# adrelino/mv-lm-icp

Hardware: NVIDIA H100
Metric: ICP iterations/sec (corr+LM) (higher is better)
Workload: dtype f64

## Files before the change

mv_lm_icp_b200/csrc/lm_step.cuh:

```cuda
#pragma once
#include <cuda_runtime.h>
#include "../../include/mvicp.h"
#include "se3_math.cuh"
#include "types.cuh"

namespace mv {

constexpr int STEP_THREADS = 512;
constexpr int EOUT = 160;

struct LmState {
  mvicp_lm_options opt;
  int32_t param, cost_kind, robust, M, E, F, n, G;
  int32_t phase, done, termination, iteration, n_success, n_invalid, n_evals, n_solves, reuse_diagonal, nonrigid;
  double radius, decrease_factor, x_cost, cand_cost, x_norm, initial_cost, model_cost_change, step_norm, gmax;
};

struct NormalLayout {
  const int32_t* col;
  const int32_t* hb_ptr; const int32_t* hb_row; const int32_t* hb_col; const int32_t* hc_edge; const int32_t* hc_sub; int32_t n_hblocks;
  const int32_t* gb_ptr; const int32_t* gc_edge; const int32_t* gc_side;
  const int32_t* rlast; const int32_t* rfirst;
  const int32_t* rowbase;
  double *Lg, *rhs;
  int32_t l_in_smem;
};

struct LmWork {
  LmState* S;
  const EdgeDev* edges;
  const double* eout;
  volatile int* peer_flags;
  int32_t world, xseq;
  double* x;
  double* cand;
  Rt* Rt_eval;
  double* K_eval;
  FrameGen* G_eval;
  double* poses16;
  volatile int32_t* host_flag;
  int32_t seq;
  long long* prof;
};

struct LmProblem {
  LmState* S;
  const int32_t* frame;
  const int32_t* edge;
  NormalLayout lay;
  double *H, *g, *Hc, *gc, *scale, *diag, *step;
};

__device__ __forceinline__ double block_sum(double v, double* red) {
  __syncthreads();
  const int lane = threadIdx.x & 31, wid = threadIdx.x >> 5;
#pragma unroll
  for (int o = 16; o > 0; o >>= 1) v += __shfl_down_sync(0xffffffffu, v, o);
  if (lane == 0) red[wid] = v;
  __syncthreads();
  if (threadIdx.x == 0) { double s = 0; for (int w = 0; w < STEP_THREADS / 32; ++w) s += red[w]; red[32] = s; }
  __syncthreads();
  return red[32];
}
__device__ __forceinline__ double block_max(double v, double* red) {
  __syncthreads();
  const int lane = threadIdx.x & 31, wid = threadIdx.x >> 5;
#pragma unroll
  for (int o = 16; o > 0; o >>= 1) v = fmax(v, __shfl_down_sync(0xffffffffu, v, o));
  if (lane == 0) red[wid] = v;
  __syncthreads();
  if (threadIdx.x == 0) { double s = 0; for (int w = 0; w < STEP_THREADS / 32; ++w) s = fmax(s, red[w]); red[32] = s; }
  __syncthreads();
  return red[32];
}

__device__ __forceinline__ void gather_blocks(const NormalLayout& l, const double* eout, int n, double* H) {
  for (int idx = threadIdx.x; idx < l.n_hblocks * 36; idx += blockDim.x) {
    const int b = idx / 36, r = idx - 36 * b, i = r / 6, j = r - 6 * i;
    double s = 0;
    for (int c = l.hb_ptr[b]; c < l.hb_ptr[b + 1]; ++c) {
      const int e = l.hc_edge[c], sub = l.hc_sub[c];
      s += eout[(size_t)EOUT * e + (6 * (sub >> 1) + i) * 12 + 6 * (sub & 1) + j];
    }
    H[(size_t)(l.hb_row[b] + i) * n + l.hb_col[b] + j] = s;
  }
}
__device__ __forceinline__ void gather_gradient(const NormalLayout& l, const double* eout, int M, double* g) {
  for (int idx = threadIdx.x; idx < M * 6; idx += blockDim.x) {
    const int f = idx / 6, i = idx - 6 * f;
    if (l.col[f] < 0) continue;
    double s = 0;
    for (int c = l.gb_ptr[f]; c < l.gb_ptr[f + 1]; ++c) s += eout[(size_t)EOUT * l.gc_edge[c] + 144 + 6 * l.gc_side[c] + i];
    g[l.col[f] + i] = s;
  }
}
__device__ __forceinline__ double edge_cost_sum(const double* eout, int E, double* red, const int32_t* edge = nullptr) {
  double s = 0.0;
  for (int e = threadIdx.x; e < E; e += blockDim.x) s += eout[(size_t)EOUT * (edge ? edge[e] : e) + 156];
  return block_sum(s, red);
}
template <typename State> __device__ __forceinline__ void copy_state(State* dst, const State* src) {
  for (int i = threadIdx.x; i < (int)(sizeof(State) / sizeof(int32_t)); i += blockDim.x)
    reinterpret_cast<int32_t*>(dst)[i] = reinterpret_cast<const int32_t*>(src)[i];
  __syncthreads();
}
__device__ __forceinline__ void publish_step(volatile int32_t* host_flag, int32_t seq, bool done) {
  __threadfence();
  host_flag[seq & 7] = (seq << 1) | (done ? 1 : 0);
  __threadfence_system();
}

__global__ void lm_init_kernel(LmWork w) {
  LmState* S = w.S;
  const int f = blockIdx.x * blockDim.x + threadIdx.x;
  if (f >= S->M) return;
  double x[7] = {0, 0, 0, 0, 0, 0, 0};
  param_of_pose(S->param, w.poses16 + 16 * f, x);
  if (S->param != PARAM_AA) {
    const double n2 = x[0] * x[0] + x[1] * x[1] + x[2] * x[2] + x[3] * x[3];
    if (!(fabs(n2 - 1.0) <= 1e-9)) atomicExch(&S->nonrigid, 1);
  }
  Rt a; Rt_of_param(S->param, x, &a);
  double K[36]; tangent_map(S->param, x, &a, K);
  for (int i = 0; i < 7; ++i) { w.x[7 * f + i] = x[i]; w.cand[7 * f + i] = x[i]; }
  w.Rt_eval[f] = a;
  for (int i = 0; i < 36; ++i) w.K_eval[36 * f + i] = K[i];
  if (w.G_eval && S->param != PARAM_AA) frame_general(S->param, x, &w.G_eval[f]);
}

__device__ __forceinline__ void chol_factor_diag(double* L, const int32_t* rb, int j0, double* dinv, volatile int* s_ok, int lane) {
  double D[6][6], inv[6];
#pragma unroll
  for (int i = 0; i < 6; ++i)
#pragma unroll
    for (int k = 0; k <= i; ++k) D[i][k] = L[rb[j0 + i] + j0 + k];
  bool okb = true;
#pragma unroll
  for (int k = 0; k < 6; ++k) {
    double d = D[k][k];
#pragma unroll
    for (int m = 0; m < k; ++m) d -= D[k][m] * D[k][m];
    if (!(d > 0.0) || !isfinite(d)) okb = false;
    inv[k] = rsqrt(d); D[k][k] = d * inv[k];
#pragma unroll
    for (int i = k + 1; i < 6; ++i) {
      double v = D[i][k];
#pragma unroll
      for (int m = 0; m < k; ++m) v -= D[i][m] * D[k][m];
      D[i][k] = v * inv[k];
    }
  }
  __syncwarp();
  if (lane == 0) {
    if (!okb) *s_ok = 0;
#pragma unroll
    for (int i = 0; i < 6; ++i) {
#pragma unroll
      for (int k = 0; k <= i; ++k) L[rb[j0 + i] + j0 + k] = D[i][k];
      dinv[j0 + i] = inv[i];
    }
  }
}

__device__ bool chol_solve(double* L, const int32_t* __restrict__ rowbase, int n, double* scratch, double* dinv, double* y,
                           const int32_t* __restrict__ rlast, const int32_t* __restrict__ rfirst, long long* prof = nullptr) {
  const int T = blockDim.x, tid = threadIdx.x, lane = tid & 31, wid = tid >> 5, nw = T >> 5;
  int32_t* s_rfirst = reinterpret_cast<int32_t*>(scratch);
  int32_t* s_rlast = s_rfirst + n;
  int32_t* rb = s_rlast + n;
  volatile int* s_ok = reinterpret_cast<volatile int*>(rb + n + 1);
  for (int i = tid; i < n; i += T) { s_rfirst[i] = rfirst[i]; s_rlast[i] = rlast[i]; }
  for (int i = tid; i <= n; i += T) rb[i] = rowbase[i];
  if (tid == 0) *s_ok = 1;
  __syncthreads();
  const int NB = n / 6;
  if (wid == 0) chol_factor_diag(L, rb, 0, dinv, s_ok, lane);
  __syncthreads();
  long long t_panel = 0, t_ahead = 0, t_bar = 0;
  for (int J = 0; J < NB; ++J) {
    if (!*s_ok) return false;
    const long long c0 = prof ? clock64() : 0;
    const int j0 = 6 * J;
    const int rl = s_rlast[j0 + 5];
    const int nrows = rl - (j0 + 5) + 1;
    for (int q = tid; q < nrows; q += T) {
      const int r = (q == nrows - 1) ? n : j0 + 6 + q;
      if (r < n && s_rfirst[r] > j0 + 5) continue;
      double* row = L + rb[r] + j0;
      double v[6];
#pragma unroll
      for (int k = 0; k < 6; ++k) {
        double a = row[k];
#pragma unroll
        for (int m = 0; m < k; ++m) a -= v[m] * L[rb[j0 + k] + j0 + m];
        v[k] = a * dinv[j0 + k];
      }
#pragma unroll
      for (int k = 0; k < 6; ++k) row[k] = v[k];
    }
    const long long c1 = prof ? clock64() : 0;
    __syncthreads();
    const long long c2 = prof ? clock64() : 0;
    const bool next = J + 1 < NB;
    if (wid == 0 && next) {
      const int b0 = j0 + 6;
      if (lane < 21 && s_rfirst[b0] <= j0 + 5) {
        int i = 0, rem = lane; while (rem > i) { rem -= i + 1; ++i; }
        const int k = rem;
        double* row = L + rb[b0 + i]; const double* lc = L + rb[b0 + k] + j0;
        double a = row[b0 + k];
#pragma unroll
        for (int m = 0; m < 6; ++m) a -= row[j0 + m] * lc[m];
        row[b0 + k] = a;
      }
      __syncwarp();
      chol_factor_diag(L, rb, b0, dinv, s_ok, lane);
    } else {
      const int w0 = next ? 1 : 0, wn = next ? nw - 1 : nw;
      const int qfirst = next ? 6 : 0;
      for (int q = qfirst + (wid - w0); q < nrows; q += wn) {
        const int r = (q == nrows - 1) ? n : j0 + 6 + q;
        if (r < n && s_rfirst[r] > j0 + 5) continue;
        double* row = L + rb[r];
        double lr[6];
#pragma unroll
        for (int k = 0; k < 6; ++k) lr[k] = row[j0 + k];
        const int cend = min(r, rl);
        for (int c = j0 + 6 + lane; c <= cend; c += 32) {
          if (s_rfirst[c] > j0 + 5) continue;
          const double* lc = L + rb[c] + j0;
          double a = row[c];
#pragma unroll
          for (int k = 0; k < 6; ++k) a -= lr[k] * lc[k];
          row[c] = a;
        }
      }
    }
    const long long c3 = prof ? clock64() : 0;
    __syncthreads();
    if (prof) { const long long c4 = clock64(); t_panel += c1 - c0; t_ahead += c3 - c2; t_bar += (c2 - c1) + (c4 - c3); }
  }
  if (prof && tid == 0) { prof[8] = t_panel; prof[9] = t_ahead; prof[10] = t_bar; }
  if (!*s_ok) return false;
  for (int i = tid; i < n; i += T) y[i] = L[rb[n] + i];
  __syncthreads();
  if (wid == 0) {
    for (int J = NB - 1; J >= 0; --J) {
      const int j0 = 6 * J;
      double x[6];
#pragma unroll
      for (int k = 5; k >= 0; --k) {
        double a = y[j0 + k];
#pragma unroll
        for (int m = k + 1; m < 6; ++m) a -= L[rb[j0 + m] + j0 + k] * x[m];
        x[k] = a * dinv[j0 + k];
      }
      __syncwarp();
#pragma unroll
      for (int k = 0; k < 6; ++k) if (lane == k) y[j0 + k] = x[k];
      for (int i = s_rfirst[j0] + lane; i < j0; i += 32) {
        double a = y[i];
#pragma unroll
        for (int k = 0; k < 6; ++k) a -= L[rb[j0 + k] + i] * x[k];
        y[i] = a;
      }
      __syncwarp();
    }
  }
  __syncthreads();
  return true;
}

__device__ __forceinline__ void lm_step_body(const LmWork& w, const LmProblem& p) {
  extern __shared__ double smem[];
  __shared__ double red[40];
  __shared__ int s_flag;
  if (p.S->done) return;
  const int tid = threadIdx.x, T = blockDim.x;
  __shared__ LmState s_state;
  copy_state(&s_state, p.S);
  LmState* S = &s_state;
  const int n = S->n, M = S->M, E = S->E, param = S->param;
  const NormalLayout& lay = p.lay;
  long long* prof = w.prof ? w.prof + 16 * (w.seq & 3) : nullptr;
#define MV_STAMP(i) do { if (prof && tid == 0) prof[i] = clock64(); } while (0)
  MV_STAMP(0);
  if (w.peer_flags) {
    if (tid < w.world) {
      const long long t0 = clock64();
      while (w.peer_flags[tid] - w.xseq < 0) {
        if (clock64() - t0 > 4000000000LL) { S->nonrigid = 2; break; }
      }
    }
    __syncthreads();
  }
  double* colj = smem; double* dg = smem + 2 * (S->n + 1);
  double* L = lay.l_in_smem ? smem + 3 * (S->n + 1) : lay.Lg;

  gather_blocks(lay, w.eout, n, p.Hc);
  gather_gradient(lay, w.eout, M, p.gc);
  __syncthreads();
  const double eval_cost = edge_cost_sum(w.eout, E, red, p.edge);

  MV_STAMP(1);
  bool take = false;
  if (tid == 0) {
    s_flag = 0;
    S->n_evals += 1;
    if (!isfinite(eval_cost)) {
      if (S->phase == 0) { S->done = 1; S->termination = MVICP_TERM_EVAL_FAILURE; }
      else {
        S->n_invalid += 1;
        if (S->n_invalid >= S->opt.max_num_consecutive_invalid_steps) { S->done = 1; S->termination = MVICP_TERM_INVALID_STEPS; }
        S->radius = S->radius / S->decrease_factor; S->decrease_factor *= 2.0; S->reuse_diagonal = 1;
      }
    } else if (S->phase == 0) {
      S->x_cost = eval_cost; S->initial_cost = eval_cost; s_flag = 1;
    } else {
      S->cand_cost = eval_cost;
      if (S->step_norm <= S->opt.parameter_tolerance * (S->x_norm + S->opt.parameter_tolerance)) {
        S->done = 1; S->termination = MVICP_TERM_PARAMETER_TOLERANCE;
      } else if (fabs(S->x_cost - eval_cost) <= S->opt.function_tolerance * S->x_cost) {
        S->done = 1; S->termination = MVICP_TERM_FUNCTION_TOLERANCE;
      } else {
        const double rho = (S->x_cost - eval_cost) / S->model_cost_change;
        if (rho > S->opt.min_relative_decrease) {
          s_flag = 1; S->n_success += 1; S->x_cost = eval_cost;
          const double q = 2.0 * rho - 1.0;
          S->radius = fmin(S->opt.max_trust_region_radius, S->radius / fmax(1.0 / 3.0, 1.0 - q * q * q));
          S->decrease_factor = 2.0; S->reuse_diagonal = 0;
        } else {
          S->radius = S->radius / S->decrease_factor; S->decrease_factor *= 2.0; S->reuse_diagonal = 1;
          if (S->radius < S->opt.min_trust_region_radius) { S->done = 1; S->termination = MVICP_TERM_MIN_RADIUS; }
        }
      }
    }
  }
  __syncthreads();
  take = s_flag != 0;
  if (take) {
    for (int idx = tid; idx < lay.n_hblocks * 36; idx += T) {
      const int b = idx / 36, r = idx - 36 * b, i = r / 6, j = r - 6 * i;
      const size_t at = (size_t)(lay.hb_row[b] + i) * n + lay.hb_col[b] + j;
      p.H[at] = p.Hc[at];
    }
    for (int idx = tid; idx < n; idx += T) p.g[idx] = p.gc[idx];
    for (int idx = tid; idx < M * 7; idx += T) { const int at = 7 * p.frame[idx / 7] + idx % 7; w.x[at] = w.cand[at]; }
    __syncthreads();
    if (S->phase == 0)
      for (int j = tid; j < n; j += T) p.scale[j] = S->opt.jacobi_scaling ? 1.0 / (1.0 + sqrt(p.H[(size_t)j * n + j])) : 1.0;
    double xs = 0.0, gm = 0.0;
    for (int f = tid; f < M; f += T) {
      if (lay.col[f] < 0) continue;
      const int G = S->G;
      double xf[7], ng[6], xp[7];
      for (int i = 0; i < G; ++i) { xf[i] = w.x[7 * p.frame[f] + i]; xs += xf[i] * xf[i]; }
      for (int i = 0; i < 6; ++i) ng[i] = -p.g[lay.col[f] + i];
      param_plus(param, xf, ng, xp);
      for (int i = 0; i < G; ++i) gm = fmax(gm, fabs(xf[i] - xp[i]));
    }
    xs = block_sum(xs, red);
    gm = block_max(gm, red);
    if (tid == 0) {
      S->x_norm = sqrt(xs); S->gmax = gm;
      if (gm <= S->opt.gradient_tolerance) { S->done = 1; S->termination = MVICP_TERM_GRADIENT_TOLERANCE; }
      if (S->phase == 0) { S->phase = 1; S->iteration = 0; S->reuse_diagonal = 0; }
    }
    __syncthreads();
  }

  MV_STAMP(2);
  while (!S->done) {
    __syncthreads();
    if (S->iteration >= S->opt.max_num_iterations) {
      __syncthreads();
      if (tid == 0) { S->done = 1; S->termination = MVICP_TERM_MAX_ITERATIONS; }
      __syncthreads();
      break;
    }
    const int reuse = S->reuse_diagonal;
    const double radius = S->radius;
    __syncthreads();
    if (!reuse)
      for (int j = tid; j < n; j += T) {
        const double d = p.scale[j] * p.scale[j] * p.H[(size_t)j * n + j];
        p.diag[j] = fmin(fmax(d, S->opt.min_lm_diagonal), S->opt.max_lm_diagonal);
      }
    __syncthreads();
    for (int i = tid >> 5; i < n; i += T >> 5) {
      const double si = p.scale[i];
      const int rbi = lay.rowbase[i];
      for (int j = lay.rfirst[i] + (tid & 31); j <= i; j += 32) {
        double v = si * p.H[(size_t)i * n + j] * p.scale[j];
        if (i == j) { const double ldg = sqrt(p.diag[i] / radius); v += ldg * ldg; }
        L[rbi + j] = v;
      }
    }
    { const int rbn = lay.rowbase[n]; for (int j = tid; j < n; j += T) L[rbn + j] = p.scale[j] * p.g[j]; }
    __syncthreads();
    MV_STAMP(3);
    bool ok = chol_solve(L, lay.rowbase, n, colj, dg, lay.rhs, lay.rlast, lay.rfirst, prof);
    MV_STAMP(4);
    double bad = 0.0;
    if (ok) for (int j = tid; j < n; j += T) if (!isfinite(lay.rhs[j])) bad = 1.0;
    bad = block_sum(bad, red);
    ok = ok && (bad == 0.0);
    double mcc = 0.0;
    if (ok) {
      for (int j = tid; j < n; j += T) p.step[j] = -lay.rhs[j];
      __syncthreads();
      double acc = 0.0;
      for (int i = tid; i < n; i += T) {
        const double y = lay.rhs[i];
        acc += 0.5 * (y * p.scale[i] * p.g[i] + (p.diag[i] / radius) * y * y);
      }
      mcc = block_sum(acc, red);
    }
    const bool valid = ok && (mcc > 0.0);
    __syncthreads();
    if (tid == 0) {
      S->iteration += 1; S->n_solves += 1; S->reuse_diagonal = 1; S->model_cost_change = mcc;
      if (!valid) {
        S->n_invalid += 1;
        if (S->n_invalid >= S->opt.max_num_consecutive_invalid_steps) { S->done = 1; S->termination = MVICP_TERM_INVALID_STEPS; }
        S->radius = S->radius / S->decrease_factor; S->decrease_factor *= 2.0;
      } else S->n_invalid = 0;
    }
    __syncthreads();
    if (!valid) continue;
    double sn = 0.0;
    for (int f = tid; f < M; f += T) {
      const int G = S->G, g_f = __ldg(p.frame + f);
      double xf[7], d[6], xp[7] = {0, 0, 0, 0, 0, 0, 0};
      for (int i = 0; i < 7; ++i) xf[i] = w.x[7 * g_f + i];
      if (lay.col[f] >= 0) {
        for (int i = 0; i < 6; ++i) d[i] = p.step[lay.col[f] + i] * p.scale[lay.col[f] + i];
        param_plus(param, xf, d, xp);
        for (int i = 0; i < G; ++i) sn += (xf[i] - xp[i]) * (xf[i] - xp[i]);
      } else for (int i = 0; i < 7; ++i) xp[i] = xf[i];
      for (int i = 0; i < 7; ++i) w.cand[7 * g_f + i] = xp[i];
      Rt a; Rt_of_param(param, xp, &a);
      w.Rt_eval[g_f] = a;
      double K[36]; tangent_map(param, xp, &a, K);
      for (int i = 0; i < 36; ++i) w.K_eval[36 * g_f + i] = K[i];
      if (w.G_eval && param != PARAM_AA) frame_general(param, xp, &w.G_eval[g_f]);
    }
    sn = block_sum(sn, red);
    MV_STAMP(5);
    if (tid == 0) S->step_norm = sqrt(sn);
    __syncthreads();
    break;
  }
  __syncthreads();
  if (S->done) {
    for (int f = tid; f < M; f += T) {
      double xf[7]; for (int i = 0; i < 7; ++i) xf[i] = w.x[7 * p.frame[f] + i];
      pose_of_param(param, xf, w.poses16 + 16 * p.frame[f]);
    }
  }
  __syncthreads();
  copy_state(p.S, &s_state);
  MV_STAMP(6);
#undef MV_STAMP
}

__global__ void __launch_bounds__(STEP_THREADS) lm_step_kernel(LmWork w, const LmProblem* __restrict__ probs, unsigned int* ticket) {
  __shared__ LmProblem s_prob;
  copy_state(&s_prob, probs + blockIdx.x);
  lm_step_body(w, s_prob);
  __shared__ int s_last;
  __syncthreads();
  int open;
  if (gridDim.x == 1) {
    open = *(volatile const int*)&s_prob.S->done == 0;
  } else {
    if (threadIdx.x == 0) { __threadfence(); s_last = atomicAdd(ticket, 1u) == gridDim.x - 1; }
    __syncthreads();
    if (!s_last) return;
    __threadfence();
    open = 0;
    for (int k = threadIdx.x; k < (int)gridDim.x; k += blockDim.x) open |= *(volatile const int*)&probs[k].S->done == 0;
    open = __syncthreads_count(open);
  }
  if (threadIdx.x == 0) {
    *ticket = 0u; publish_step(w.host_flag, w.seq, open == 0);
    if (w.prof) w.prof[16 * (w.seq & 3) + 7] = clock64();
  }
}

}
```

Before: 565.8.

## Unroll gathers, fuse block reductions, and stage back-substitution in shared memory

Gradient and Hessian gathers now have each thread process two indices together, so their irregular loads overlap. Two pairs of back-to-back block reductions become a single dual reduction, which removes barriers. The Cholesky back-substitution now works on a shared-memory copy of the right-hand side and hoists row-base offsets into registers. The finiteness check, step write and model-cost accumulation are fused into one pass. The shared scratch layout is reshuffled, which risks aliasing between ys (placed at scratch+n+1 as doubles) and the int32 index arrays.

```diff
diff --git a/mv_lm_icp_b200/csrc/lm_step.cuh b/mv_lm_icp_b200/csrc/lm_step.cuh
--- a/mv_lm_icp_b200/csrc/lm_step.cuh
+++ b/mv_lm_icp_b200/csrc/lm_step.cuh
@@ -73,25 +73,86 @@
   __syncthreads();
   return red[32];
 }
-
+__device__ __forceinline__ void block_reduce2(double& a, double& b, bool b_max, double* red) {
+  __syncthreads();
+  const int lane = threadIdx.x & 31, wid = threadIdx.x >> 5;
+#pragma unroll
+  for (int o = 16; o > 0; o >>= 1) {
+    a += __shfl_down_sync(0xffffffffu, a, o);
+    const double t = __shfl_down_sync(0xffffffffu, b, o);
+    b = b_max ? fmax(b, t) : b + t;
+  }
+  if (lane == 0) { red[wid] = a; red[STEP_THREADS / 32 + wid] = b; }
+  __syncthreads();
+  if (threadIdx.x == 0) {
+    double s = 0, m = 0;
+    for (int w = 0; w < STEP_THREADS / 32; ++w) { s += red[w]; m = b_max ? fmax(m, red[STEP_THREADS / 32 + w]) : m + red[STEP_THREADS / 32 + w]; }
+    red[32] = s; red[33] = m;
+  }
+  __syncthreads();
+  a = red[32]; b = red[33];
+}
+
+constexpr int GATHER_U = 2;
 __device__ __forceinline__ void gather_blocks(const NormalLayout& l, const double* eout, int n, double* H) {
-  for (int idx = threadIdx.x; idx < l.n_hblocks * 36; idx += blockDim.x) {
-    const int b = idx / 36, r = idx - 36 * b, i = r / 6, j = r - 6 * i;
-    double s = 0;
-    for (int c = l.hb_ptr[b]; c < l.hb_ptr[b + 1]; ++c) {
-      const int e = l.hc_edge[c], sub = l.hc_sub[c];
-      s += eout[(size_t)EOUT * e + (6 * (sub >> 1) + i) * 12 + 6 * (sub & 1) + j];
-    }
-    H[(size_t)(l.hb_row[b] + i) * n + l.hb_col[b] + j] = s;
+  const int total = l.n_hblocks * 36, T = blockDim.x;
+  for (int base = threadIdx.x; base < total; base += GATHER_U * T) {
+    int c0[GATHER_U], c1[GATHER_U], ij[GATHER_U], row[GATHER_U], col[GATHER_U]; double s[GATHER_U];
+#pragma unroll
+    for (int u = 0; u < GATHER_U; ++u) {
+      const int idx = base + u * T;
+      c0[u] = c1[u] = 0; ij[u] = row[u] = col[u] = 0; s[u] = 0;
+      if (idx < total) {
+        const int b = idx / 36, r = idx - 36 * b, i = r / 6, j = r - 6 * i;
+        c0[u] = l.hb_ptr[b]; c1[u] = l.hb_ptr[b + 1]; ij[u] = i * 12 + j;
+        row[u] = l.hb_row[b] + i; col[u] = l.hb_col[b] + j;
+      }
+    }
+    for (int k = 0;; ++k) {
+      bool more = false;
+#pragma unroll
+      for (int u = 0; u < GATHER_U; ++u) more |= c0[u] + k < c1[u];
+      if (!more) break;
+      int e[GATHER_U], sub[GATHER_U];
+#pragma unroll
+      for (int u = 0; u < GATHER_U; ++u)
+        if (c0[u] + k < c1[u]) { e[u] = l.hc_edge[c0[u] + k]; sub[u] = l.hc_sub[c0[u] + k]; }
+#pragma unroll
+      for (int u = 0; u < GATHER_U; ++u)
+        if (c0[u] + k < c1[u]) s[u] += eout[(size_t)EOUT * e[u] + 72 * (sub[u] >> 1) + ij[u] + 6 * (sub[u] & 1)];
+    }
+#pragma unroll
+    for (int u = 0; u < GATHER_U; ++u) if (base + u * T < total) H[(size_t)row[u] * n + col[u]] = s[u];
   }
 }
 __device__ __forceinline__ void gather_gradient(const NormalLayout& l, const double* eout, int M, double* g) {
-  for (int idx = threadIdx.x; idx < M * 6; idx += blockDim.x) {
-    const int f = idx / 6, i = idx - 6 * f;
-    if (l.col[f] < 0) continue;
-    double s = 0;
-    for (int c = l.gb_ptr[f]; c < l.gb_ptr[f + 1]; ++c) s += eout[(size_t)EOUT * l.gc_edge[c] + 144 + 6 * l.gc_side[c] + i];
-    g[l.col[f] + i] = s;
+  const int total = M * 6, T = blockDim.x;
+  for (int base = threadIdx.x; base < total; base += GATHER_U * T) {
+    int c0[GATHER_U], c1[GATHER_U], iu[GATHER_U], at[GATHER_U]; double s[GATHER_U];
+#pragma unroll
+    for (int u = 0; u < GATHER_U; ++u) {
+      const int idx = base + u * T;
+      c0[u] = c1[u] = 0; iu[u] = 0; at[u] = -1; s[u] = 0;
+      if (idx < total) {
+        const int f = idx / 6, i = idx - 6 * f, col = l.col[f];
+        if (col >= 0) { c0[u] = l.gb_ptr[f]; c1[u] = l.gb_ptr[f + 1]; iu[u] = i; at[u] = col + i; }
+      }
+    }
+    for (int k = 0;; ++k) {
+      bool more = false;
+#pragma unroll
+      for (int u = 0; u < GATHER_U; ++u) more |= c0[u] + k < c1[u];
+      if (!more) break;
+      int e[GATHER_U], side[GATHER_U];
+#pragma unroll
+      for (int u = 0; u < GATHER_U; ++u)
+        if (c0[u] + k < c1[u]) { e[u] = l.gc_edge[c0[u] + k]; side[u] = l.gc_side[c0[u] + k]; }
+#pragma unroll
+      for (int u = 0; u < GATHER_U; ++u)
+        if (c0[u] + k < c1[u]) s[u] += eout[(size_t)EOUT * e[u] + 144 + 6 * side[u] + iu[u]];
+    }
+#pragma unroll
+    for (int u = 0; u < GATHER_U; ++u) if (at[u] >= 0) g[at[u]] = s[u];
   }
 }
 __device__ __forceinline__ double edge_cost_sum(const double* eout, int E, double* red, const int32_t* edge = nullptr) {
@@ -130,10 +191,13 @@
 
 __device__ __forceinline__ void chol_factor_diag(double* L, const int32_t* rb, int j0, double* dinv, volatile int* s_ok, int lane) {
   double D[6][6], inv[6];
+  int at[6];
+#pragma unroll
+  for (int i = 0; i < 6; ++i) at[i] = rb[j0 + i] + j0;
 #pragma unroll
   for (int i = 0; i < 6; ++i)
 #pragma unroll
-    for (int k = 0; k <= i; ++k) D[i][k] = L[rb[j0 + i] + j0 + k];
+    for (int k = 0; k <= i; ++k) D[i][k] = L[at[i] + k];
   bool okb = true;
 #pragma unroll
   for (int k = 0; k < 6; ++k) {
@@ -156,7 +220,7 @@
 #pragma unroll
     for (int i = 0; i < 6; ++i) {
 #pragma unroll
-      for (int k = 0; k <= i; ++k) L[rb[j0 + i] + j0 + k] = D[i][k];
+      for (int k = 0; k <= i; ++k) L[at[i] + k] = D[i][k];
       dinv[j0 + i] = inv[i];
     }
   }
@@ -165,10 +229,11 @@
 __device__ bool chol_solve(double* L, const int32_t* __restrict__ rowbase, int n, double* scratch, double* dinv, double* y,
                            const int32_t* __restrict__ rlast, const int32_t* __restrict__ rfirst, long long* prof = nullptr) {
   const int T = blockDim.x, tid = threadIdx.x, lane = tid & 31, wid = tid >> 5, nw = T >> 5;
-  int32_t* s_rfirst = reinterpret_cast<int32_t*>(scratch);
-  int32_t* s_rlast = s_rfirst + n;
-  int32_t* rb = s_rlast + n;
-  volatile int* s_ok = reinterpret_cast<volatile int*>(rb + n + 1);
+  int32_t* rb = reinterpret_cast<int32_t*>(scratch);
+  int32_t* s_rfirst = rb + n + 1;
+  volatile int* s_ok = reinterpret_cast<volatile int*>(s_rfirst + n);
+  int32_t* s_rlast = s_rfirst + n + 1;
+  double* ys = scratch + n + 1;
   for (int i = tid; i < n; i += T) { s_rfirst[i] = rfirst[i]; s_rlast[i] = rlast[i]; }
   for (int i = tid; i <= n; i += T) rb[i] = rowbase[i];
   if (tid == 0) *s_ok = 1;
@@ -242,31 +307,37 @@
   }
   if (prof && tid == 0) { prof[8] = t_panel; prof[9] = t_ahead; prof[10] = t_bar; }
   if (!*s_ok) return false;
-  for (int i = tid; i < n; i += T) y[i] = L[rb[n] + i];
+  for (int i = tid; i < n; i += T) ys[i] = L[rb[n] + i];
   __syncthreads();
   if (wid == 0) {
     for (int J = NB - 1; J >= 0; --J) {
       const int j0 = 6 * J;
+      int at[6];
+#pragma unroll
+      for (int k = 0; k < 6; ++k) at[k] = rb[j0 + k];
+      const int i0 = s_rfirst[j0];
       double x[6];
 #pragma unroll
       for (int k = 5; k >= 0; --k) {
-        double a = y[j0 + k];
-#pragma unroll
-        for (int m = k + 1; m < 6; ++m) a -= L[rb[j0 + m] + j0 + k] * x[m];
+        double a = ys[j0 + k];
+#pragma unroll
+        for (int m = k + 1; m < 6; ++m) a -= L[at[m] + j0 + k] * x[m];
         x[k] = a * dinv[j0 + k];
       }
       __syncwarp();
 #pragma unroll
-      for (int k = 0; k < 6; ++k) if (lane == k) y[j0 + k] = x[k];
-      for (int i = s_rfirst[j0] + lane; i < j0; i += 32) {
-        double a = y[i];
-#pragma unroll
-        for (int k = 0; k < 6; ++k) a -= L[rb[j0 + k] + i] * x[k];
-        y[i] = a;
+      for (int k = 0; k < 6; ++k) if (lane == k) ys[j0 + k] = x[k];
+      for (int i = i0 + lane; i < j0; i += 32) {
+        double a = ys[i];
+#pragma unroll
+        for (int k = 0; k < 6; ++k) a -= L[at[k] + i] * x[k];
+        ys[i] = a;
       }
       __syncwarp();
     }
   }
+  __syncthreads();
+  for (int i = tid; i < n; i += T) y[i] = ys[i];
   __syncthreads();
   return true;
 }
@@ -339,10 +410,17 @@
   __syncthreads();
   take = s_flag != 0;
   if (take) {
-    for (int idx = tid; idx < lay.n_hblocks * 36; idx += T) {
-      const int b = idx / 36, r = idx - 36 * b, i = r / 6, j = r - 6 * i;
-      const size_t at = (size_t)(lay.hb_row[b] + i) * n + lay.hb_col[b] + j;
-      p.H[at] = p.Hc[at];
+    for (int base = tid, total = lay.n_hblocks * 36; base < total; base += GATHER_U * T) {
+      size_t at[GATHER_U]; double v[GATHER_U];
+#pragma unroll
+      for (int u = 0; u < GATHER_U; ++u) {
+        const int idx = base + u * T, b = idx / 36, r = idx - 36 * b, i = r / 6, j = r - 6 * i;
+        at[u] = idx < total ? (size_t)(lay.hb_row[b] + i) * n + lay.hb_col[b] + j : 0;
+      }
+#pragma unroll
+      for (int u = 0; u < GATHER_U; ++u) if (base + u * T < total) v[u] = p.Hc[at[u]];
+#pragma unroll
+      for (int u = 0; u < GATHER_U; ++u) if (base + u * T < total) p.H[at[u]] = v[u];
     }
     for (int idx = tid; idx < n; idx += T) p.g[idx] = p.gc[idx];
     for (int idx = tid; idx < M * 7; idx += T) { const int at = 7 * p.frame[idx / 7] + idx % 7; w.x[at] = w.cand[at]; }
@@ -359,8 +437,7 @@
       param_plus(param, xf, ng, xp);
       for (int i = 0; i < G; ++i) gm = fmax(gm, fabs(xf[i] - xp[i]));
     }
-    xs = block_sum(xs, red);
-    gm = block_max(gm, red);
+    block_reduce2(xs, gm, true, red);
     if (tid == 0) {
       S->x_norm = sqrt(xs); S->gmax = gm;
       if (gm <= S->opt.gradient_tolerance) { S->done = 1; S->termination = MVICP_TERM_GRADIENT_TOLERANCE; }
@@ -401,21 +478,17 @@
     MV_STAMP(3);
     bool ok = chol_solve(L, lay.rowbase, n, colj, dg, lay.rhs, lay.rlast, lay.rfirst, prof);
     MV_STAMP(4);
-    double bad = 0.0;
-    if (ok) for (int j = tid; j < n; j += T) if (!isfinite(lay.rhs[j])) bad = 1.0;
-    bad = block_sum(bad, red);
-    ok = ok && (bad == 0.0);
-    double mcc = 0.0;
-    if (ok) {
-      for (int j = tid; j < n; j += T) p.step[j] = -lay.rhs[j];
-      __syncthreads();
-      double acc = 0.0;
+    double bad = 0.0, mcc = 0.0;
+    if (ok)
       for (int i = tid; i < n; i += T) {
         const double y = lay.rhs[i];
-        acc += 0.5 * (y * p.scale[i] * p.g[i] + (p.diag[i] / radius) * y * y);
-      }
-      mcc = block_sum(acc, red);
-    }
+        if (!isfinite(y)) bad = 1.0;
+        p.step[i] = -y;
+        mcc += 0.5 * (y * p.scale[i] * p.g[i] + (p.diag[i] / radius) * y * y);
+      }
+    block_reduce2(bad, mcc, false, red);
+    ok = ok && (bad == 0.0);
+    if (!ok) mcc = 0.0;
     const bool valid = ok && (mcc > 0.0);
     __syncthreads();
     if (tid == 0) {
```

Result: faster. 573.1, median of 6 (+1.3%).
